# nicoloalbergoni/DeepLabV3Plus-Augmented-SuperResolution

Measured on AMD Instinct MI355X. Metric: augmented-copies/sec (fwd+realign+SR-iter) @512x512, higher is better.
Workload: dtype f32 (pointwise GEMMs: operands split into f16 hi+lo, hi*hi+hi*lo+lo*hi on f16 MFMA, f32 accumulate)

## Files before the change

### deeplabv3plus-augmented-superresolution_amd/csrc/sr.hip

```cpp
#include "asr_warp_device.h"

namespace {

constexpr int kTileX = 32, kTileY = 8;

struct SrDims {
    int batch, n, H, W, h, w, f;
};

__global__ __launch_bounds__(256) void sr_init_kernel(const float* __restrict__ y, float* __restrict__ x,
                                                      SrDims d, float scale_y, float scale_x) {
    const int X = blockIdx.x * kTileX + threadIdx.x;
    const int Y = blockIdx.y * kTileY + threadIdx.y;
    const int b = blockIdx.z;
    if (X >= d.W || Y >= d.H) return;
    const float* src = y + (int64_t)b * d.n * d.h * d.w;
    const AsrLerp ly = asr_half_pixel(Y, scale_y, d.h);
    const AsrLerp lx = asr_half_pixel(X, scale_x, d.w);
    const float tl = src[ly.lo * d.w + lx.lo], tr = src[ly.lo * d.w + lx.hi];
    const float bl = src[ly.hi * d.w + lx.lo], br = src[ly.hi * d.w + lx.hi];
    const float top = tl + (tr - tl) * lx.t;
    const float bot = bl + (br - bl) * lx.t;
    x[((int64_t)b * d.H + Y) * d.W + X] = top + (bot - top) * ly.t;
}

#if defined(ASR_DIAG_KFWD_CHECK) || defined(ASR_DIAG_KFWD_NOPK)
__device__ __forceinline__ float dg_mul(float x, float y) { float z; asm volatile("v_mul_f32 %0, %1, %2" : "=v"(z) : "v"(x), "v"(y)); return z; }
__device__ __forceinline__ float dg_add(float x, float y) { float z; asm volatile("v_add_f32 %0, %1, %2" : "=v"(z) : "v"(x), "v"(y)); return z; }
__device__ __forceinline__ float dg_sub(float x, float y) { float z; asm volatile("v_sub_f32 %0, %1, %2" : "=v"(z) : "v"(x), "v"(y)); return z; }
#endif
#ifndef ASR_DIAG_KFWD_NOPK
#define ASR_DIAG_KFWD_NOPK 0
#endif
constexpr int kGrPadX = 32, kGrPadY = 2;
__host__ __device__ inline size_t sr_gr_plane_elems(int H, int W) { return (size_t)(H + 2 * kGrPadY) * (size_t)(W + 2 * kGrPadX); }
typedef float asr_f2u __attribute__((ext_vector_type(2), aligned(4)));

__device__ __forceinline__ float sr_bilinear_bordered(const float* __restrict__ plane, int WP, int H, int W, float ix, float iy) {
    const float xf = floorf(ix), yf = floorf(iy);
    const int x0 = (int)__builtin_amdgcn_fmed3f(xf, -2.0f, (float)W), y0 = (int)__builtin_amdgcn_fmed3f(yf, -2.0f, (float)H);
    const unsigned off = (unsigned)(__mul24(y0, WP * 4) + (kGrPadY * WP * 4 + kGrPadX * 4) + x0 * 4);
    const char* const base = reinterpret_cast<const char*>(plane);
    const char* const base_next = base + WP * 4;
    const asr_f2u top = *reinterpret_cast<const asr_f2u*>(base + off);
    const asr_f2u bot = *reinterpret_cast<const asr_f2u*>(base_next + off);
#ifdef ASR_DIAG_KFWD_WAIT
    asm volatile("s_waitcnt vmcnt(0)" ::: "memory");
#endif
#if ASR_DIAG_KFWD_NOPK & 2
    const float wxl = dg_sub(dg_add(xf, 1.0f), ix), wxh = dg_sub(ix, xf);
    const float vyf = dg_add(dg_mul(wxl, top.x), dg_mul(wxh, top.y));
    const float vyc = dg_add(dg_mul(wxl, bot.x), dg_mul(wxh, bot.y));
    return dg_add(dg_mul(dg_sub(dg_add(yf, 1.0f), iy), vyf), dg_mul(dg_sub(iy, yf), vyc));
// ... 282 lines not shown
            const float acc = v[o] + g * g;
            v[o] = acc;
            xn = xc - (g * alpha) / (sqrtf(acc) + st.c2);
            break;
        }
        case ASR_OPT_ADADELTA: {
            const float acc = v[o] * st.c0 + (g * g) * st.c1;
            v[o] = acc;
            const float au = m[o];
            const float upd = sqrtf(au + st.c2) * (1.0f / sqrtf(acc + st.c2)) * g;
            xn = xc - upd * alpha;
            m[o] = au * st.c0 + (upd * upd) * st.c1;
            break;
        }
        case ASR_OPT_ADAMAX: {
            float mm = m[o];
            mm = mm + (g - mm) * st.c0;
            const float vv = fmaxf(st.c1 * v[o], fabsf(g));
            m[o] = mm;
            v[o] = vv;
            xn = xc - alpha * (mm / (vv + st.c2));
            break;
        }
        default: {
            float mm = m[o], vv = v[o];
            mm = mm + (g - mm) * st.c0;
            vv = vv + (g * g - vv) * st.c1;
            m[o] = mm;
            v[o] = vv;
            float denom;
            if (st.flag) {
                const float vh = fmaxf(vhat[o], vv);
                vhat[o] = vh;
                denom = sqrtf(vh) + st.c2;
            } else {
                denom = sqrtf(vv) + st.c2;
            }
            xn = xc - (mm * alpha) / denom;
        }
    }
    x_new[o] = xn;
    if (x_bordered_out)
        x_bordered_out[(size_t)b * sr_gr_plane_elems(H, W) + (size_t)(Y + kGrPadY) * (W + 2 * kGrPadX) + (X + kGrPadX)] = xn;
}

constexpr int kBwdSplit = 4, kBwdPixX = 32, kBwdPixY = 2, kBwdPix = kBwdPixX * kBwdPixY;

constexpr int kGrRows = 16;

template <int LOG2F>
__global__ __launch_bounds__(256) void sr_grad_translate_kernel(const float* __restrict__ resid,
                                                                const float* __restrict__ inv_trans_tf,
                                                                float* __restrict__ gr_out, SrDims d, float two_lambda_df,
                                                                int n0, int cn) {
    const int slot = blockIdx.z;
    const int bn = (slot / cn) * d.n + n0 + (slot % cn);
    const int lane = threadIdx.x;
    const int cx = blockIdx.x * 64 + lane;
    const int cy0 = (blockIdx.y * 4 + __builtin_amdgcn_readfirstlane(threadIdx.y)) * kGrRows;
    const int H = d.H, W = d.W, f = d.f, lw = d.w, lh = d.h;
    const int ph0 = f / 2 - 1, ph1 = f / 2;
    const int WP = W + 2 * kGrPadX;
    const float* r = resid + (int64_t)bn * lh * lw;
    const AsrTf8 it = asr_load_tf(inv_trans_tf + (int64_t)bn * 8);
    float* const out = gr_out + (size_t)slot * sr_gr_plane_elems(H, W) + (size_t)kGrPadY * WP + kGrPadX;
    const bool col_ok = cx < W;
    const bool pure_translation = (it.a0 == 1.0f && it.a1 == 0.0f && it.b0 == 0.0f && it.b1 == 1.0f &&
                                   it.c0 == 0.0f && it.c1 == 0.0f);
    if (pure_translation) {
        const SrAxisTap ax = sr_axis_tap<LOG2F>(col_ok ? cx : 0, it.a2, W, f, ph0, ph1);
        const int c0 = max(ax.l0, 0), c1 = max(ax.l1, 0);
        const bool ok0 = ax.l0 >= 0, ok1 = ax.l1 >= 0;
        const SrAxisTap ayv = sr_axis_tap<LOG2F>(min(cy0 + lane, H - 1), it.b2, H, f, ph0, ph1);
        auto xblend = [&](int L) -> float {
            const float* row = r + L * lw;
            const float a = (two_lambda_df * row[c0]) * 0.25f, b = (two_lambda_df * row[c1]) * 0.25f;
            return ax.wl * (ok0 ? a : 0.0f) + ax.wh * (ok1 ? b : 0.0f);
        };
        int la = -1, lb = -1;
        float va = 0.0f, vb = 0.0f;
        auto h_of = [&](int L) -> float {
            if (L < 0) return 0.0f;
            if (L == lb) return vb;
            if (L == la) return va;
            la = lb; va = vb;
            lb = L; vb = xblend(L);
            return vb;
        };
        const int rows = min(kGrRows, H - cy0);
        for (int j = 0; j < rows; ++j) {
            const float wl = __builtin_bit_cast(float, __builtin_amdgcn_readlane(__builtin_bit_cast(int, ayv.wl), j));
            const float wh = __builtin_bit_cast(float, __builtin_amdgcn_readlane(__builtin_bit_cast(int, ayv.wh), j));
            const int l0 = __builtin_amdgcn_readlane(ayv.l0, j), l1 = __builtin_amdgcn_readlane(ayv.l1, j);
            const float h0 = h_of(l0), h1 = h_of(l1);
            if (col_ok) out[(cy0 + j) * WP + cx] = wl * h0 + wh * h1;
        }
    } else {
        auto gt_at = [&](int ly, int lx) -> float {
            const bool ok = (ly >= 0) & (lx >= 0);
            const float v = (two_lambda_df * r[ok ? ly * lw + lx : 0]) * 0.25f;
            return ok ? v : 0.0f;
        };
        auto rd_gt = [&](int yt, int xt) -> float {
            return gt_at(sr_gt_index<LOG2F>(yt, H, f, ph0, ph1), sr_gt_index<LOG2F>(xt, W, f, ph0, ph1));
        };
        for (int j = 0; j < kGrRows; ++j) {
            const int cy = cy0 + j;
            if (cy < H && col_ok) out[cy * WP + cx] = asr_tf_sample(it, rd_gt, cx, cy);
        }
    }
}

template <int LOG2F, bool WTV>
__global__ __launch_bounds__(256) void sr_backward_adam_kernel(
    const float* __restrict__ x, float* __restrict__ x_new, const float* __restrict__ resid,
    const float* __restrict__ inv_rot_tf, const float* __restrict__ inv_trans_tf,
    float* __restrict__ m, float* __restrict__ v, float* __restrict__ vhat,
    const float* __restrict__ alphas , float* __restrict__ grad_out,
    SrDims d, float two_lambda_df, float lambda_tv, float two_lambda_l2, float lambda_l1, SrStep st, SrTvW tw) {
    extern __shared__ float contrib[];
    const int X = blockIdx.x * kBwdPixX + threadIdx.x;
    const int Y = blockIdx.y * kBwdPixY + threadIdx.y;
    const int b = blockIdx.z;
    const int grp = threadIdx.z;
    const int pix = threadIdx.y * kBwdPixX + threadIdx.x;
    const bool in_image = (X < d.W) & (Y < d.H);
    const int H = d.H, W = d.W, f = d.f, lw = d.w, lh = d.h;
    const int ph0 = f / 2 - 1, ph1 = f / 2;

    auto contribution = [&](int n) -> float {
        float g_df = 0.0f;
        const int bn = b * d.n + n;
        const AsrTf8 ir = asr_load_tf(inv_rot_tf + (int64_t)bn * 8);
        const float* r = resid + (int64_t)bn * lh * lw;
        const AsrTf8 it = asr_load_tf(inv_trans_tf + (int64_t)bn * 8);
        auto gt_at = [&](int ly, int lx) -> float {
            const bool ok = (ly >= 0) & (lx >= 0);
            const float v = (two_lambda_df * r[ok ? ly * lw + lx : 0]) * 0.25f;
            return ok ? v : 0.0f;
        };
        const bool pure_translation = (it.a0 == 1.0f && it.a1 == 0.0f && it.b0 == 0.0f && it.b1 == 1.0f &&
                                       it.c0 == 0.0f && it.c1 == 0.0f);
        if (pure_translation) {
// ... 109 lines not shown
    for (int i = threadIdx.x; i < n; i += 64) {
        const float* t = inv_rot_tf + ((int64_t)b * n + i) * 8;
        ok = ok && t[6] == 0.0f && t[7] == 0.0f;
    }
    const bool all = __builtin_amdgcn_ballot_w64(!ok) == 0;
    if (threadIdx.x == 0) flags[b] = all ? 1 : 0;
}

template <bool WTV>
__global__ __launch_bounds__(256) void sr_backward_gather_kernel(
    const float* __restrict__ x, float* __restrict__ x_new, const float* __restrict__ gr_planes,
    const float* __restrict__ inv_rot_tf, float* __restrict__ m, float* __restrict__ v, float* __restrict__ vhat,
    const float* __restrict__ alphas, float* __restrict__ grad_out, SrDims d, float lambda_tv, float two_lambda_l2,
    float lambda_l1, SrStep st, float* __restrict__ x_bordered_out, float* __restrict__ acc, int n0, int cn,
    const int* __restrict__ affine_flags, SrTvW tw) {
    const int X = blockIdx.x * 64 + threadIdx.x;
    const int Y = blockIdx.y * 4 + threadIdx.y;
    const int b = blockIdx.z;
    const int H = d.H, W = d.W, WP = W + 2 * kGrPadX;
    if (X >= W || Y >= H) return;
    const size_t plane = sr_gr_plane_elems(H, W);
    const float* const planes = gr_planes + (size_t)b * cn * plane;
    const float* const tfs = inv_rot_tf + ((int64_t)b * d.n + n0) * 8;
    const float fx = (float)X, fy = (float)Y;
    const int64_t o = ((int64_t)b * H + Y) * W + X;
    float g_df = (n0 == 0) ? 0.0f : acc[o];
    int n = 0;
    if (affine_flags[b]) {
        for (; n + 8 <= cn; n += 8) g_df = sr_gather_chunk<8, true>(g_df, tfs + n * 8, planes + n * plane, plane, WP, H, W, fx, fy);
        if (n + 4 <= cn) { g_df = sr_gather_chunk<4, true>(g_df, tfs + n * 8, planes + n * plane, plane, WP, H, W, fx, fy); n += 4; }
        for (; n < cn; ++n) g_df = sr_gather_chunk<1, true>(g_df, tfs + n * 8, planes + n * plane, plane, WP, H, W, fx, fy);
    } else {
        for (; n < cn; ++n) g_df = sr_gather_chunk<1, false>(g_df, tfs + n * 8, planes + n * plane, plane, WP, H, W, fx, fy);
    }
    if (n0 + cn < d.n) { acc[o] = g_df; return; }
    sr_prior_and_update<WTV>(x, x_new, m, v, vhat, alphas, grad_out, d, b, X, Y, g_df, lambda_tv, two_lambda_l2, lambda_l1, st,
                             tw, x_bordered_out);
}

typedef void (*SrBwdKernel)(const float*, float*, const float*, const float*, const float*, float*, float*, float*,
                            const float*, float*, SrDims, float, float, float, float, SrStep, SrTvW);

template <bool WTV>
SrBwdKernel sr_backward_kernel_of(int f) {
    switch (f) {
        case 2: return sr_backward_adam_kernel<1, WTV>;
        case 4: return sr_backward_adam_kernel<2, WTV>;
        case 8: return sr_backward_adam_kernel<3, WTV>;
        default: return sr_backward_adam_kernel<0, WTV>;
    }
}
SrBwdKernel sr_backward_kernel_for(int f, bool wtv) { return wtv ? sr_backward_kernel_of<true>(f) : sr_backward_kernel_of<false>(f); }

typedef void (*SrGradTranslateKernel)(const float*, const float*, float*, SrDims, float, int, int);
SrGradTranslateKernel sr_grad_translate_kernel_for(int f) {
    switch (f) {
        case 2: return sr_grad_translate_kernel<1>;
        case 4: return sr_grad_translate_kernel<2>;
        case 8: return sr_grad_translate_kernel<3>;
        default: return sr_grad_translate_kernel<0>;
    }
}

__global__ __launch_bounds__(256) void sr_loss_df_kernel(const float* __restrict__ resid, double* __restrict__ out,
                                                         int64_t per_image) {
    const int b = blockIdx.y;
    const float* r = resid + (int64_t)b * per_image;
    double acc = 0.0;
    for (int64_t p = (int64_t)blockIdx.x * 256 + threadIdx.x; p < per_image; p += (int64_t)gridDim.x * 256) {
        const float t = r[p];
        acc += (double)(t * t);
    }
    acc = asr_wave_sum(acc);
    if ((threadIdx.x & 63) == 0) atomicAdd(out + (int64_t)b * 4 + 0, acc);
}

template <bool WTV>
__global__ __launch_bounds__(256) void sr_loss_prior_kernel(const float* __restrict__ x, double* __restrict__ out,
                                                            int H, int W, SrStep st, SrTvW tw) {
    const int b = blockIdx.y;
    const float* img = x + (int64_t)b * H * W;
    double tv = 0.0, l2 = 0.0, l1 = 0.0;
    const int64_t total = (int64_t)H * W;
    for (int64_t p = (int64_t)blockIdx.x * 256 + threadIdx.x; p < total; p += (int64_t)gridDim.x * 256) {
        const int X = (int)(p % W), Y = (int)(p / W);
        const float xc = img[p];
        if (st.prior == ASR_PRIOR_BTV) {
            for (int hh = -st.btv_shift; hh <= st.btv_shift; ++hh)
                for (int vv = 0; vv <= st.btv_shift; ++vv) {
                    const int xs = X - hh, ys = Y - vv;
                    const float sv = (xs >= 0 && xs < W && ys >= 0 && ys < H) ? img[(int64_t)ys * W + xs] : 0.0f;
                    tv += (double)st.btv_w[abs(hh) + vv] * (double)fabsf(xc - sv);
                }
        } else if (WTV) {
            const float dy = (Y < H - 1) ? img[p + W] - xc : 0.0f;
            const float dx = (X < W - 1) ? img[p + 1] - xc : 0.0f;
            const int64_t q = (int64_t)b * tw.stride + p;
            tv += (double)(tw.wy[q] * fabsf(dy) + tw.wx[q] * fabsf(dx));
        } else {
            const float dy = (Y < H - 1) ? img[p + W] - xc : 0.0f;
            const float dx = (X < W - 1) ? img[p + 1] - xc : 0.0f;
            tv += (double)(fabsf(dy) + fabsf(dx));
        }
        l2 += (double)(xc * xc);
        l1 += (double)fabsf(xc);
    }
    tv = asr_wave_sum(tv);
// ... 67 lines not shown
    };
    V val;
    float ix, iy;
    const bool ok = asr_tf_map(tr, (float)X, (float)Y, ix, iy);
    const float xf = floorf(ix), yf = floorf(iy);
    const int x0 = asr_coord_to_int(xf), y0 = asr_coord_to_int(yf);
    const bool pure_translation = (tt.a0 == 1.0f) & (tt.a1 == 0.0f) & (tt.b0 == 0.0f) & (tt.b1 == 1.0f) &
                                  (tt.c0 == 0.0f) & (tt.c1 == 0.0f);
    const float jx0 = (float)x0 + tt.a2, jx1 = (float)(x0 + 1) + tt.a2;
    const float jy0 = (float)y0 + tt.b2, jy1 = (float)(y0 + 1) + tt.b2;
    const float fx0 = floorf(jx0), fx1 = floorf(jx1), fy0 = floorf(jy0), fy1 = floorf(jy1);
    const int cx0 = asr_coord_to_int(fx0), cx1 = asr_coord_to_int(fx1);
    const int cy0 = asr_coord_to_int(fy0), cy1 = asr_coord_to_int(fy1);
    if (ok && pure_translation && cx1 == cx0 + 1 && cy1 == cy0 + 1) {
        V uv[3][3];
#pragma unroll
        for (int a = 0; a < 3; ++a)
#pragma unroll
            for (int c = 0; c < 3; ++c) uv[a][c] = rd_up(cy0 + a, cx0 + c);
        const float wxl0 = (fx0 + 1.0f) - jx0, wxh0 = jx0 - fx0, wxl1 = (fx1 + 1.0f) - jx1, wxh1 = jx1 - fx1;
        const float wyl0 = (fy0 + 1.0f) - jy0, wyh0 = jy0 - fy0, wyl1 = (fy1 + 1.0f) - jy1, wyh1 = jy1 - fy1;
        auto Tq = [&](int a, int c, float wxl, float wxh, float wyl, float wyh) -> V {
            const V vyf = wxl * uv[a][c] + wxh * uv[a][c + 1];
            const V vyc = wxl * uv[a + 1][c] + wxh * uv[a + 1][c + 1];
            return wyl * vyf + wyh * vyc;
        };
        const bool vx0 = x0 >= 0 && x0 < W, vx1 = x0 + 1 >= 0 && x0 + 1 < W;
        const bool vy0 = y0 >= 0 && y0 < H, vy1 = y0 + 1 >= 0 && y0 + 1 < H;
        const V v00 = (vy0 && vx0) ? Tq(0, 0, wxl0, wxh0, wyl0, wyh0) : zero;
        const V v01 = (vy0 && vx1) ? Tq(0, 1, wxl1, wxh1, wyl0, wyh0) : zero;
        const V v10 = (vy1 && vx0) ? Tq(1, 0, wxl0, wxh0, wyl1, wyh1) : zero;
        const V v11 = (vy1 && vx1) ? Tq(1, 1, wxl1, wxh1, wyl1, wyh1) : zero;
        const float wxl = (xf + 1.0f) - ix, wxh = ix - xf;
        const V vyf = wxl * v00 + wxh * v01;
        const V vyc = wxl * v10 + wxh * v11;
        val = ((yf + 1.0f) - iy) * vyf + (iy - yf) * vyc;
    } else {
        val = asr_tf_sample(tr, rd_tr, X, Y);
    }
    return val;
}
__device__ __forceinline__ float sr_realign_copy_value(const float* __restrict__ y, const float* __restrict__ trans_tf,
                                                       const float* __restrict__ rot_tf, int bn, int X, int Y, int H, int W,
                                                       int lh, int lw, float scale_y, float scale_x) {
    const float* const src[1] = {y + (int64_t)bn * lh * lw};
    return sr_realign_copy_value<1>(src, trans_tf, rot_tf, bn, X, Y, H, W, lh, lw, scale_y, scale_x).v[0];
}

template <int MODE>
__global__ __launch_bounds__(256) void sr_realign_kernel(const float* __restrict__ y, float* __restrict__ out_a,
                                                         float* __restrict__ out_b,
                                                         const float* __restrict__ trans_tf ,
                                                         const float* __restrict__ rot_tf ,
                                                         SrDims d, float scale_y, float scale_x) {
    const int X = blockIdx.x * kTileX + threadIdx.x;
    const int Y = blockIdx.y * kTileY + threadIdx.y;
    const int b = blockIdx.z;
    if (X >= d.W || Y >= d.H) return;
    const int H = d.H, W = d.W, lh = d.h, lw = d.w;
    float acc_sum = 0.0f, acc_max = 0.0f;
    for (int n = 0; n < d.n; ++n) {
        const float val = sr_realign_copy_value(y, trans_tf, rot_tf, b * d.n + n, X, Y, H, W, lh, lw, scale_y, scale_x);
        if (MODE != 0) acc_max = (n == 0) ? val : fmaxf(acc_max, val);
        if (MODE != 1) acc_sum += val;
    }
    const int64_t o = ((int64_t)b * H + Y) * W + X;
    if (MODE == 0) out_a[o] = acc_sum / (float)d.n;
    if (MODE == 1) out_a[o] = acc_max;
    if (MODE == 2) { out_a[o] = acc_max; out_b[o] = acc_sum / (float)d.n; }
}

constexpr int kSelX = 32, kSelY = 2, kSelPix = kSelX * kSelY;
constexpr int kSelMaxQ = 8;
constexpr int kSelLdsMax = 160 * 1024;
constexpr int kSelMaxCopies = kSelLdsMax / (kSelPix * (int)sizeof(unsigned));

struct SrSelect {
    int num_q, trim_k;
    int lo[kSelMaxQ], hi[kSelMaxQ];
    float t[kSelMaxQ];
};

__device__ __forceinline__ unsigned sr_sel_key(float v) {
    const unsigned u = __float_as_uint(v == 0.0f ? 0.0f : v);
    return u ^ ((u >> 31) ? 0xffffffffu : 0x80000000u);
}
__device__ __forceinline__ float sr_sel_value(unsigned k) {
    return __uint_as_float(k ^ ((k >> 31) ? 0x80000000u : 0xffffffffu));
}
__device__ __forceinline__ unsigned sr_sel_rank(const unsigned* col, int n, int rank) {
    unsigned prefix = 0u;
    for (int bit = 31; bit >= 0; --bit) {
        const unsigned cand = prefix | (1u << bit);
        int below = 0;
#pragma unroll 8
        for (int i = 0; i < n; ++i) below += (col[i * kSelPix] < cand) ? 1 : 0;
        prefix = (below <= rank) ? cand : prefix;
    }
    return prefix;
}

__global__ __launch_bounds__(kSelPix) void sr_realign_select_kernel(const float* __restrict__ y, float* __restrict__ out_q,
                                                                    float* __restrict__ out_trim,
                                                                    const float* __restrict__ trans_tf,
                                                                    const float* __restrict__ rot_tf, SrDims d, SrSelect sel,
                                                                    int tiles_x, float scale_y, float scale_x) {
    extern __shared__ unsigned sel_keys[];
    const int tile_y = blockIdx.x / tiles_x, tile_x = blockIdx.x - tile_y * tiles_x;
    const int X = tile_x * kSelX + threadIdx.x;
    const int Y = tile_y * kSelY + threadIdx.y;
    const int b = blockIdx.z;
    if (X >= d.W || Y >= d.H) return;
    const int H = d.H, W = d.W, lh = d.h, lw = d.w, n = d.n;
    unsigned* col = sel_keys + threadIdx.y * kSelX + threadIdx.x;
    for (int i = 0; i < n; ++i) {
        const float val = sr_realign_copy_value(y, trans_tf, rot_tf, b * n + i, X, Y, H, W, lh, lw, scale_y, scale_x);
        col[i * kSelPix] = sr_sel_key(val);
    }
    const int64_t plane = (int64_t)d.batch * H * W;
    const int64_t o = ((int64_t)b * H + Y) * W + X;
    for (int j = 0; j < sel.num_q; ++j) {
        const int lo = sel.lo[j], hi = sel.hi[j];
// ... 155 lines not shown
        if (walk == 0) {
            fnv = (float)cnt;
            m = (cnt > 0) ? acc / fnv : 0.0f;
            if (out_nv) out_nv[o] = fnv;
            if (out_mean) out_mean[o] = m;
        } else {
            out_var[o] = (fnv > 0.0f) ? acc / fnv : 0.0f;
        }
    }
}

int check_dims(const char* fn, int batch, int n, int H, int W, int h, int w, SrDims* d) {
    ASR_REQUIRE(batch > 0 && n > 0 && H > 0 && W > 0 && h > 0 && w > 0, "%s: bad shape batch=%d n=%d %dx%d <- %dx%d",
                fn, batch, n, H, W, h, w);
    ASR_REQUIRE((int64_t)batch * n <= 65535, "%s: batch*n=%lld exceeds 65535 (grid.z)", fn, (long long)batch * n);
    const int f = H / h;
    ASR_UNSUPPORTED(f * h != H || f * w != W || f < 2 || (f & 1),
                    "%s: output %dx%d must be an even integer multiple of the feature size %dx%d", fn, H, W, h, w);
    d->batch = batch; d->n = n; d->H = H; d->W = W; d->h = h; d->w = w; d->f = f;
    return ASR_OK;
}

int prepare_backward(const SrDims& d, bool wtv) {
    const size_t lds = sizeof(float) * (size_t)d.n * 64;
    ASR_UNSUPPORTED(lds > 160 * 1024, "asr_sr: num_aug=%d needs %zu bytes of LDS in the backward kernel (max 640 copies)", d.n, lds);
    static AsrDeviceOnce once[8];
    const int idx = (d.f == 2 ? 1 : (d.f == 4 ? 2 : (d.f == 8 ? 3 : 0))) + (wtv ? 4 : 0);
    if (lds > 64 * 1024)
        ASR_HIP_CHECK(asr_allow_dynamic_lds(once[idx], reinterpret_cast<const void*>(sr_backward_kernel_for(d.f, wtv)), 160 * 1024));
    return ASR_OK;
}
dim3 gr_grid(const SrDims& d, int cn) {
    return dim3((unsigned)asr_cdiv(d.W, 64), (unsigned)asr_cdiv(d.H, 4 * kGrRows), (unsigned)(d.batch * cn));
}
constexpr size_t kPlaneBytesMax = (size_t)1 << 30;
int sr_plane_chunk(int batch, int n, int H, int W, int requested) {
    if (requested > 0) return requested < n ? requested : n;
    const size_t per_copy = sizeof(float) * (size_t)batch * sr_gr_plane_elems(H, W);
    const size_t fit = kPlaneBytesMax / per_copy > 0 ? kPlaneBytesMax / per_copy : 1;
    if ((size_t)n <= fit) return n;
    const int chunks = (int)(((size_t)n + fit - 1) / fit);
    return (n + chunks - 1) / chunks;
}
size_t sr_workspace_bytes(int batch, int n, int H, int W, int h, int w, int chunk) {
    return sizeof(float) * ((size_t)batch * n * h * w + 2 * (size_t)batch * H * W +
                            ((size_t)batch * chunk + batch) * sr_gr_plane_elems(H, W)) + sizeof(int) * (size_t)batch;
}
dim3 gather_grid(const SrDims& d) {
    return dim3((unsigned)asr_cdiv(d.W, 64), (unsigned)asr_cdiv(d.H, 4), (unsigned)d.batch);
}
dim3 bwd_grid(const SrDims& d) { return dim3((unsigned)asr_cdiv(d.W, kBwdPixX), (unsigned)asr_cdiv(d.H, kBwdPixY), (unsigned)d.batch); }
const dim3 kBwdBlock(kBwdPixX, kBwdPixY, kBwdSplit);
size_t bwd_lds(const SrDims& d) { return sizeof(float) * (size_t)d.n * kBwdPix; }
dim3 hr_grid(const SrDims& d) { return dim3((unsigned)asr_cdiv(d.W, kTileX), (unsigned)asr_cdiv(d.H, kTileY), (unsigned)d.batch); }
dim3 lr_grid(const SrDims& d) { return dim3((unsigned)asr_cdiv(d.w, kTileX), (unsigned)asr_cdiv(d.h, kTileY), (unsigned)(d.batch * d.n)); }
const dim3 kBlock(kTileX, kTileY);

}

extern "C" int asr_sr_init_target_f32(const float* y, float* x, int batch, int n, int H, int W, int h, int w,
                                      asr_stream_t stream) {
    ASR_REQUIRE(y && x, "asr_sr_init_target_f32: null pointer");
    SrDims d;
    ASR_REQUIRE(batch > 0 && n > 0 && H > 0 && W > 0 && h > 0 && w > 0, "asr_sr_init_target_f32: bad shape");
    d.batch = batch; d.n = n; d.H = H; d.W = W; d.h = h; d.w = w; d.f = 0;
    const float sy = (float)h / (float)H, sx = (float)w / (float)W;
    hipLaunchKernelGGL(sr_init_kernel, hr_grid(d), kBlock, 0, asr_stream(stream), y, x, d, sy, sx);
    ASR_LAUNCH_CHECK();
    return ASR_OK;
}

extern "C" int asr_sr_forward_residual_f32(const float* x, const float* y, const float* rot_tf, const float* trans_tf,
                                           float* resid, int batch, int n, int H, int W, int h, int w,
                                           asr_stream_t stream) {
    ASR_REQUIRE(x && y && rot_tf && trans_tf && resid, "asr_sr_forward_residual_f32: null pointer");
    SrDims d;
    int rc = check_dims("asr_sr_forward_residual_f32", batch, n, H, W, h, w, &d);
    if (rc != ASR_OK) return rc;
    hipLaunchKernelGGL(sr_forward_residual_kernel<false>, lr_grid(d), kBlock, 0, asr_stream(stream), x, y, rot_tf, trans_tf,
                       resid, d);
    ASR_LAUNCH_CHECK();
    return ASR_OK;
}

namespace {

int make_step(const char* fn, const asr_sr_config* cfg, bool need_update, const float* m, const float* v, const float* vhat,
              SrStep* st) {
    ASR_REQUIRE(cfg, "%s: null config", fn);
    ASR_REQUIRE(cfg->optimizer >= ASR_OPT_ADAM && cfg->optimizer <= ASR_OPT_ADAMAX, "%s: unknown optimizer %d", fn, cfg->optimizer);
    ASR_REQUIRE(cfg->prior == ASR_PRIOR_TV || cfg->prior == ASR_PRIOR_BTV, "%s: unknown prior %d", fn, cfg->prior);
    st->optimizer = cfg->optimizer; st->flag = cfg->flag; st->c0 = cfg->c0; st->c1 = cfg->c1; st->c2 = cfg->c2;
    st->prior = cfg->prior; st->btv_shift = 0;
    for (int k = 0; k < 9; ++k) st->btv_w[k] = 0.0f;
    if (cfg->prior == ASR_PRIOR_BTV) {
        ASR_REQUIRE(cfg->btv_shift >= 1 && cfg->btv_shift <= 4, "%s: btv_shift %d outside [1, 4]", fn, cfg->btv_shift);
        st->btv_shift = cfg->btv_shift;
        for (int k = 0; k <= 2 * cfg->btv_shift; ++k) st->btv_w[k] = powf(cfg->btv_alpha, (float)k);
    }
    if (need_update) {
        bool ok = true;
        switch (cfg->optimizer) {
            case ASR_OPT_ADAM: ok = m && v && (vhat || !cfg->flag); break;
            case ASR_OPT_SGD: ok = m || cfg->c0 == 0.0f; break;
            case ASR_OPT_ADAGRAD: ok = v != nullptr; break;
            default: ok = m && v; break;
// ... 122 lines not shown
extern "C" int asr_sr_loss_terms_f64(const float* x, const float* resid, double* terms, int batch, int n, int H, int W,
                                     int h, int w, asr_stream_t stream) {
    const asr_sr_config c = adam_tv_config(0.f, 0.f, 0.f, 0);
    return asr_sr_loss_terms_cfg_f64(x, resid, terms, batch, n, H, W, h, w, &c, stream);
}

extern "C" size_t asr_sr_solve_workspace_bytes(int batch, int n, int H, int W, int h, int w) {
    return sr_workspace_bytes(batch, n, H, W, h, w, sr_plane_chunk(batch, n, H, W, 0));
}

extern "C" size_t asr_sr_solve_workspace_bytes_cfg(int batch, int n, int H, int W, int h, int w, const asr_sr_config* cfg) {
    return sr_workspace_bytes(batch, n, H, W, h, w, sr_plane_chunk(batch, n, H, W, cfg ? cfg->plane_chunk : 0));
}

namespace {
int sr_solve_impl(const char* fn, float* x, const float* y, const float* rot_tf, const float* trans_tf, const float* inv_rot_tf,
                  const float* inv_trans_tf, float* m, float* v, float* vhat, const float* alphas, int num_iter,
                  double* last_loss_terms, void* workspace, size_t workspace_bytes, int batch, int n, int H, int W, int h, int w,
                  float lambda_df, float lambda_tv, float lambda_l2, float lambda_l1, const asr_sr_config* cfg,
                  const SrTvWArg& wa, asr_stream_t stream) {
    ASR_REQUIRE(x && y && rot_tf && trans_tf && inv_rot_tf && inv_trans_tf && alphas && workspace, "%s: null pointer", fn);
    ASR_REQUIRE(num_iter >= 0, "%s: num_iter < 0", fn);
    SrDims d;
    int rc = check_dims(fn, batch, n, H, W, h, w, &d);
    if (rc != ASR_OK) return rc;
    SrStep st;
    rc = make_step(fn, cfg, true, m, v, vhat, &st);
    if (rc != ASR_OK) return rc;
    SrTvW tw;
    rc = make_tv_weights(fn, cfg, wa, H, W, &tw);
    if (rc != ASR_OK) return rc;
    ASR_REQUIRE(cfg->plane_chunk >= 0, "%s: plane_chunk %d < 0", fn, cfg->plane_chunk);
    const int chunk = sr_plane_chunk(batch, n, H, W, cfg->plane_chunk);
    ASR_REQUIRE((int64_t)batch * chunk <= 65535, "%s: batch*chunk=%lld exceeds 65535 (grid.z)", fn, (long long)batch * chunk);
    const size_t need = sr_workspace_bytes(batch, n, H, W, h, w, chunk);
    if (workspace_bytes < need) {
        asr_set_error("%s: workspace %zu < required %zu bytes", fn, workspace_bytes, need);
        return ASR_ERR_WORKSPACE;
    }
    hipStream_t s = asr_stream(stream);
    float* resid = static_cast<float*>(workspace);
    float* x_alt = resid + (size_t)batch * n * h * w;
    float* cur = x;
    float* nxt = x_alt;
    float* const acc = x_alt + (size_t)batch * H * W;
    float* const gr = acc + (size_t)batch * H * W;
    const SrGradTranslateKernel gr_kernel = sr_grad_translate_kernel_for(d.f);
    float* const xb = gr + (size_t)batch * chunk * sr_gr_plane_elems(H, W);
    int* const affine_flags = reinterpret_cast<int*>(xb + (size_t)batch * sr_gr_plane_elems(H, W));
    if (num_iter > 0) {
        hipLaunchKernelGGL(sr_affine_flags_kernel, dim3((unsigned)batch), dim3(64), 0, s, inv_rot_tf, affine_flags, n);
        ASR_LAUNCH_CHECK();
    }
    if (num_iter > 0) {
        const size_t pe = sr_gr_plane_elems(H, W);
        ASR_HIP_CHECK(hipMemsetAsync(gr, 0, sizeof(float) * ((size_t)batch * chunk + batch) * pe, s));
        const size_t wp = (size_t)W + 2 * kGrPadX;
        for (int b = 0; b < batch; ++b)
            ASR_HIP_CHECK(hipMemcpy2DAsync(xb + b * pe + kGrPadY * wp + kGrPadX, wp * sizeof(float), x + (size_t)b * H * W,
                                           (size_t)W * sizeof(float), (size_t)W * sizeof(float), (size_t)H,
                                           hipMemcpyDeviceToDevice, s));
    }
    for (int it = 0; it < num_iter; ++it) {
        hipLaunchKernelGGL(sr_forward_residual_kernel<true>, lr_grid(d), kBlock, 0, s, xb, y, rot_tf, trans_tf, resid, d);
        ASR_LAUNCH_CHECK();
        if (last_loss_terms && it == num_iter - 1) {
            rc = sr_loss_terms_impl(fn, cur, resid, last_loss_terms, batch, n, H, W, h, w, cfg, wa, stream);
            if (rc != ASR_OK) return rc;
        }
        for (int n0 = 0; n0 < n; n0 += chunk) {
            const int cn = n - n0 < chunk ? n - n0 : chunk;
            hipLaunchKernelGGL(gr_kernel, gr_grid(d, cn), dim3(64, 4), 0, s, resid, inv_trans_tf, gr, d, 2.0f * lambda_df, n0, cn);
            ASR_LAUNCH_CHECK();
            const auto bwd_kernel = wa.weighted ? sr_backward_gather_kernel<true> : sr_backward_gather_kernel<false>;
            hipLaunchKernelGGL(bwd_kernel, gather_grid(d), dim3(64, 4), 0, s, cur, nxt, gr, inv_rot_tf, m, v, vhat,
                               alphas + (size_t)it * batch, (float*)nullptr, d, lambda_tv, 2.0f * lambda_l2, lambda_l1, st, xb,
                               acc, n0, cn, affine_flags, tw);
            ASR_LAUNCH_CHECK();
        }
        float* t = cur; cur = nxt; nxt = t;
    }
    if (cur != x) ASR_HIP_CHECK(hipMemcpyAsync(x, cur, sizeof(float) * (size_t)batch * H * W, hipMemcpyDeviceToDevice, s));
    return ASR_OK;
}

__global__ __launch_bounds__(256) SR_NO_PK_F32 void sr_tv_edge_weights_kernel(const float* __restrict__ guide, float* __restrict__ wy,
                                                                              float* __restrict__ wx, int H, int W, float beta) {
    const int X = blockIdx.x * kTileX + threadIdx.x;
    const int Y = blockIdx.y * kTileY + threadIdx.y;
    if (X >= W || Y >= H) return;
    const int64_t o = ((int64_t)blockIdx.z * H + Y) * W + X;
    const float* c = guide + o * 3;
    const float c0 = c[0], c1 = c[1], c2 = c[2];
    float vy = 1.0f, vx = 1.0f;
    if (Y < H - 1) {
        const float* q = c + (int64_t)W * 3;
        const float a0 = q[0] - c0, a1 = q[1] - c1, a2 = q[2] - c2;
        const float dd = (a0 * a0 + a1 * a1) + a2 * a2;
        vy = 1.0f / (1.0f + beta * dd);
    }
    if (X < W - 1) {
        const float a0 = c[3] - c0, a1 = c[4] - c1, a2 = c[5] - c2;
        const float dd = (a0 * a0 + a1 * a1) + a2 * a2;
        vx = 1.0f / (1.0f + beta * dd);
    }
    wy[o] = vy;
    wx[o] = vx;
}
}

extern "C" int asr_tv_edge_weights_f32(const float* guide, float* wy, float* wx, int batch, int H, int W, float beta,
                                       asr_stream_t stream) {
    ASR_REQUIRE(guide && wy && wx, "asr_tv_edge_weights_f32: null pointer");
    ASR_REQUIRE(batch > 0 && batch <= 65535 && H > 0 && W > 0, "asr_tv_edge_weights_f32: bad shape batch=%d %dx%d", batch, H, W);
    ASR_REQUIRE(beta >= 0.0f && beta < __builtin_inff(), "asr_tv_edge_weights_f32: beta=%g must be finite and >= 0", (double)beta);
    SrDims d;
    d.batch = batch; d.n = 1; d.H = H; d.W = W; d.h = H; d.w = W; d.f = 0;
    hipLaunchKernelGGL(sr_tv_edge_weights_kernel, hr_grid(d), kBlock, 0, asr_stream(stream), guide, wy, wx, H, W, beta);
    ASR_LAUNCH_CHECK();
    return ASR_OK;
}

extern "C" int asr_sr_solve_cfg_f32(float* x, const float* y, const float* rot_tf, const float* trans_tf,
                                    const float* inv_rot_tf, const float* inv_trans_tf, float* m, float* v, float* vhat,
                                    const float* alphas, int num_iter, double* last_loss_terms, void* workspace,
                                    size_t workspace_bytes, int batch, int n, int H, int W, int h, int w,
                                    float lambda_df, float lambda_tv, float lambda_l2, float lambda_l1,
                                    const asr_sr_config* cfg, asr_stream_t stream) {
    return sr_solve_impl("asr_sr_solve_cfg_f32", x, y, rot_tf, trans_tf, inv_rot_tf, inv_trans_tf, m, v, vhat, alphas, num_iter,
                         last_loss_terms, workspace, workspace_bytes, batch, n, H, W, h, w, lambda_df, lambda_tv, lambda_l2,
                         lambda_l1, cfg, kNoTvW, stream);
}

extern "C" int asr_sr_solve_wtv_f32(float* x, const float* y, const float* rot_tf, const float* trans_tf,
                                    const float* inv_rot_tf, const float* inv_trans_tf, float* m, float* v, float* vhat,
                                    const float* alphas, int num_iter, double* last_loss_terms, void* workspace,
                                    size_t workspace_bytes, int batch, int n, int H, int W, int h, int w,
                                    float lambda_df, float lambda_tv, float lambda_l2, float lambda_l1,
                                    const asr_sr_config* cfg, const float* wy, const float* wx, int w_shared,
                                    asr_stream_t stream) {
    const SrTvWArg wa = {wy, wx, w_shared, true};
    return sr_solve_impl("asr_sr_solve_wtv_f32", x, y, rot_tf, trans_tf, inv_rot_tf, inv_trans_tf, m, v, vhat, alphas, num_iter,
                         last_loss_terms, workspace, workspace_bytes, batch, n, H, W, h, w, lambda_df, lambda_tv, lambda_l2,
                         lambda_l1, cfg, wa, stream);
}

extern "C" int asr_sr_solve_f32(float* x, const float* y, const float* rot_tf, const float* trans_tf,
                                const float* inv_rot_tf, const float* inv_trans_tf, float* m, float* v, float* vhat,
                                const float* alphas, int num_iter, double* last_loss_terms, void* workspace,
                                size_t workspace_bytes, int batch, int n, int H, int W, int h, int w,
                                float lambda_df, float lambda_tv, float lambda_l2, float lambda_l1,
                                float one_minus_beta1, float one_minus_beta2, float epsilon, int amsgrad,
                                asr_stream_t stream) {
    const asr_sr_config c = adam_tv_config(one_minus_beta1, one_minus_beta2, epsilon, amsgrad);
    return asr_sr_solve_cfg_f32(x, y, rot_tf, trans_tf, inv_rot_tf, inv_trans_tf, m, v, vhat, alphas, num_iter,
                                last_loss_terms, workspace, workspace_bytes, batch, n, H, W, h, w, lambda_df, lambda_tv,
                                lambda_l2, lambda_l1, &c, stream);
}

static int realign_common(int mode, const float* y, float* out_a, float* out_b, const float* trans_tf, const float* rot_tf,
                          int batch, int n, int H, int W, int h, int w, asr_stream_t stream) {
    ASR_REQUIRE(y && out_a && trans_tf && rot_tf && (mode != 2 || out_b), "asr_realign: null pointer");
    ASR_REQUIRE(batch > 0 && batch <= 65535 && n > 0 && H > 0 && W > 0 && h > 0 && w > 0, "asr_realign: bad shape");
    SrDims d;
    d.batch = batch; d.n = n; d.H = H; d.W = W; d.h = h; d.w = w; d.f = 0;
    const float sy = (float)h / (float)H, sx = (float)w / (float)W;
    hipStream_t s = asr_stream(stream);
    if (mode == 1) hipLaunchKernelGGL(sr_realign_kernel<1>, hr_grid(d), kBlock, 0, s, y, out_a, out_b, trans_tf, rot_tf, d, sy, sx);
    else if (mode == 0) hipLaunchKernelGGL(sr_realign_kernel<0>, hr_grid(d), kBlock, 0, s, y, out_a, out_b, trans_tf, rot_tf, d, sy, sx);
    else hipLaunchKernelGGL(sr_realign_kernel<2>, hr_grid(d), kBlock, 0, s, y, out_a, out_b, trans_tf, rot_tf, d, sy, sx);
    ASR_LAUNCH_CHECK();
    return ASR_OK;
}

extern "C" int asr_realign_max_f32(const float* y, float* out, const float* trans_tf, const float* rot_tf, int batch,
                                   int n, int H, int W, int h, int w, asr_stream_t stream) {
    return realign_common(1, y, out, nullptr, trans_tf, rot_tf, batch, n, H, W, h, w, stream);
}

extern "C" int asr_realign_mean_f32(const float* y, float* out, const float* trans_tf, const float* rot_tf, int batch,
                                    int n, int H, int W, int h, int w, asr_stream_t stream) {
    return realign_common(0, y, out, nullptr, trans_tf, rot_tf, batch, n, H, W, h, w, stream);
}

extern "C" int asr_realign_max_mean_f32(const float* y, float* out_max, float* out_mean, const float* trans_tf,
                                        const float* rot_tf, int batch, int n, int H, int W, int h, int w,
                                        asr_stream_t stream) {
    return realign_common(2, y, out_max, out_mean, trans_tf, rot_tf, batch, n, H, W, h, w, stream);
}

extern "C" int asr_realign_select_max_copies(void) { return kSelMaxCopies; }

extern "C" int asr_realign_select_f32(const float* y, float* out_q, float* out_trim, const int* lo_rank, const int* hi_rank,
                                      const float* t, int num_q, int trim_k, const float* trans_tf, const float* rot_tf,
                                      int batch, int n, int H, int W, int h, int w, asr_stream_t stream) {
    ASR_REQUIRE(y && trans_tf && rot_tf, "asr_realign_select_f32: null pointer");
    ASR_REQUIRE(num_q >= 0 && num_q <= kSelMaxQ, "asr_realign_select_f32: num_q=%d (0..%d)", num_q, kSelMaxQ);
    ASR_REQUIRE(num_q > 0 || out_trim, "asr_realign_select_f32: nothing to compute (num_q = 0 and no out_trim)");
    ASR_REQUIRE(num_q == 0 || (out_q && lo_rank && hi_rank && t), "asr_realign_select_f32: null pointer");
    ASR_REQUIRE(batch > 0 && batch <= 65535 && n > 0 && H > 0 && W > 0 && h > 0 && w > 0, "asr_realign_select_f32: bad shape");
    ASR_UNSUPPORTED(n > kSelMaxCopies, "asr_realign_select_f32: n=%d copies, at most %d (256 bytes of LDS per copy, 160 KiB per workgroup)",
                    n, kSelMaxCopies);
    SrSelect sel = {};
    sel.num_q = num_q;
    for (int j = 0; j < num_q; ++j) {
        ASR_REQUIRE(lo_rank[j] >= 0 && lo_rank[j] <= hi_rank[j] && hi_rank[j] <= n - 1,
                    "asr_realign_select_f32: ranks[%d] = (%d, %d) need 0 <= lo <= hi <= n - 1 = %d", j, lo_rank[j], hi_rank[j], n - 1);
        sel.lo[j] = lo_rank[j]; sel.hi[j] = hi_rank[j]; sel.t[j] = t[j];
    }
    ASR_REQUIRE(trim_k >= 0 && 2 * (int64_t)trim_k < n, "asr_realign_select_f32: trim_k=%d needs 0 <= 2k < n = %d", trim_k, n);
    ASR_REQUIRE(out_trim || trim_k == 0, "asr_realign_select_f32: trim_k=%d without out_trim", trim_k);
    sel.trim_k = trim_k;
    const int64_t tiles_x = asr_cdiv(W, kSelX), tiles = tiles_x * asr_cdiv(H, kSelY);
    ASR_REQUIRE(tiles <= 0x7fffffff, "asr_realign_select_f32: %dx%d output exceeds the grid", H, W);
    SrDims d;
    d.batch = batch; d.n = n; d.H = H; d.W = W; d.h = h; d.w = w; d.f = 0;
    const float sy = (float)h / (float)H, sx = (float)w / (float)W;
    const size_t lds = sizeof(unsigned) * (size_t)n * kSelPix;
    static AsrDeviceOnce once;
    if (lds > 64 * 1024)
        ASR_HIP_CHECK(asr_allow_dynamic_lds(once, reinterpret_cast<const void*>(sr_realign_select_kernel), kSelLdsMax));
    hipLaunchKernelGGL(sr_realign_select_kernel, dim3((unsigned)tiles, 1, (unsigned)batch), dim3(kSelX, kSelY), lds,
                       asr_stream(stream), y, out_q, out_trim, trans_tf, rot_tf, d, sel, (int)tiles_x, sy, sx);
    ASR_LAUNCH_CHECK();
// ... 73 lines not shown
```

Before: 2158.

## Split realign into translate-plane pass and rotation gather for translation-only batches

For batches whose transforms decompose into a pure translation followed by a rotation, realign now runs in two stages. First it materialises per-copy translated, upsampled planes with row caching into pooled scratch memory, in chunks. A gather kernel then applies the rotation with a bilinear lookup and reduces max and mean, and the original per-pixel kernel skips those batches through a flags array. The SR gradient kernel also skips output rows whose taps are all out of range when only one chunk is used. This trades redundant per-pixel composite sampling for extra scratch traffic, added launches and a stream-ordered memory pool.

```diff
diff --git a/deeplabv3plus-augmented-superresolution_amd/csrc/sr.hip b/deeplabv3plus-augmented-superresolution_amd/csrc/sr.hip
--- a/deeplabv3plus-augmented-superresolution_amd/csrc/sr.hip
+++ b/deeplabv3plus-augmented-superresolution_amd/csrc/sr.hip
@@ -1,4 +1,5 @@
 #include "asr_warp_device.h"
+#include <mutex>
 
 namespace {
 
@@ -387,7 +388,7 @@
 __global__ __launch_bounds__(256) void sr_grad_translate_kernel(const float* __restrict__ resid,
                                                                 const float* __restrict__ inv_trans_tf,
                                                                 float* __restrict__ gr_out, SrDims d, float two_lambda_df,
-                                                                int n0, int cn) {
+                                                                int n0, int cn, int skip_zero_rows) {
     const int slot = blockIdx.z;
     const int bn = (slot / cn) * d.n + n0 + (slot % cn);
     const int lane = threadIdx.x;
@@ -423,7 +424,10 @@
             return vb;
         };
         const int rows = min(kGrRows, H - cy0);
+        const unsigned long long zero_rows =
+            skip_zero_rows ? __builtin_amdgcn_ballot_w64(ayv.l0 < 0 && ayv.l1 < 0 && ayv.wl == ayv.wl && ayv.wh == ayv.wh) : 0ull;
         for (int j = 0; j < rows; ++j) {
+            if ((zero_rows >> j) & 1ull) continue;
             const float wl = __builtin_bit_cast(float, __builtin_amdgcn_readlane(__builtin_bit_cast(int, ayv.wl), j));
             const float wh = __builtin_bit_cast(float, __builtin_amdgcn_readlane(__builtin_bit_cast(int, ayv.wh), j));
             const int l0 = __builtin_amdgcn_readlane(ayv.l0, j), l1 = __builtin_amdgcn_readlane(ayv.l1, j);
@@ -639,7 +643,7 @@
 }
 SrBwdKernel sr_backward_kernel_for(int f, bool wtv) { return wtv ? sr_backward_kernel_of<true>(f) : sr_backward_kernel_of<false>(f); }
 
-typedef void (*SrGradTranslateKernel)(const float*, const float*, float*, SrDims, float, int, int);
+typedef void (*SrGradTranslateKernel)(const float*, const float*, float*, SrDims, float, int, int, int);
 SrGradTranslateKernel sr_grad_translate_kernel_for(int f) {
     switch (f) {
         case 2: return sr_grad_translate_kernel<1>;
@@ -813,11 +817,13 @@
                                                          float* __restrict__ out_b,
                                                          const float* __restrict__ trans_tf ,
                                                          const float* __restrict__ rot_tf ,
-                                                         SrDims d, float scale_y, float scale_x) {
+                                                         SrDims d, float scale_y, float scale_x,
+                                                         const int* __restrict__ plane_flags) {
     const int X = blockIdx.x * kTileX + threadIdx.x;
     const int Y = blockIdx.y * kTileY + threadIdx.y;
     const int b = blockIdx.z;
     if (X >= d.W || Y >= d.H) return;
+    if (plane_flags && plane_flags[b]) return;
     const int H = d.H, W = d.W, lh = d.h, lw = d.w;
     float acc_sum = 0.0f, acc_max = 0.0f;
     for (int n = 0; n < d.n; ++n) {
@@ -829,6 +835,179 @@
     if (MODE == 0) out_a[o] = acc_sum / (float)d.n;
     if (MODE == 1) out_a[o] = acc_max;
     if (MODE == 2) { out_a[o] = acc_max; out_b[o] = acc_sum / (float)d.n; }
+}
+
+__global__ __launch_bounds__(64) void sr_realign_flags_kernel(const float* __restrict__ trans_tf, const float* __restrict__ rot_tf,
+                                                              int* __restrict__ flags, int n) {
+    const int b = blockIdx.x;
+    bool ok = true;
+    for (int i = threadIdx.x; i < n; i += 64) {
+        const float* r = rot_tf + ((int64_t)b * n + i) * 8;
+        const float* t = trans_tf + ((int64_t)b * n + i) * 8;
+        ok = ok && r[6] == 0.0f && r[7] == 0.0f && t[0] == 1.0f && t[1] == 0.0f && t[3] == 0.0f && t[4] == 1.0f &&
+             t[6] == 0.0f && t[7] == 0.0f;
+    }
+    const bool all = __builtin_amdgcn_ballot_w64(!ok) == 0;
+    if (threadIdx.x == 0) flags[b] = all ? 1 : 0;
+}
+
+struct SrUpTap {
+    int lo, hi;
+    float t;
+    bool ok;
+};
+__device__ __forceinline__ SrUpTap sr_up_tap(int u, int size, float scale, int in_size) {
+    SrUpTap r;
+    r.ok = (u >= 0 && u < size);
+    const AsrLerp l = asr_half_pixel(r.ok ? u : 0, scale, in_size);
+    r.lo = l.lo; r.hi = l.hi; r.t = l.t;
+    return r;
+}
+
+__global__ __launch_bounds__(256) void sr_realign_planes_kernel(const float* __restrict__ y, const float* __restrict__ trans_tf,
+                                                                float* __restrict__ planes, const int* __restrict__ flags,
+                                                                SrDims d, float scale_y, float scale_x, int n0, int cn) {
+    const int slot = blockIdx.z;
+    const int b = slot / cn;
+    if (!flags[b]) return;
+    const int bn = b * d.n + n0 + (slot % cn);
+    const int lane = threadIdx.x;
+    const int cx = blockIdx.x * 64 + lane;
+    const int cy0 = (blockIdx.y * 4 + __builtin_amdgcn_readfirstlane(threadIdx.y)) * kGrRows;
+    const int H = d.H, W = d.W, lh = d.h, lw = d.w;
+    if (cy0 >= H) return;
+    const int WP = W + 2 * kGrPadX;
+    const float* const src = y + (int64_t)bn * lh * lw;
+    float* const out = planes + (size_t)slot * sr_gr_plane_elems(H, W) + (size_t)kGrPadY * WP + kGrPadX;
+    const bool col_ok = cx < W;
+    const bool col_st = cx < W + 2;
+    const int rows = min(kGrRows, H - cy0);
+    if ((int)blockIdx.x * 64 < W) {
+        const AsrTf8 tt = asr_load_tf(trans_tf + (int64_t)bn * 8);
+        const float jx = (float)(col_ok ? cx : 0) + tt.a2;
+        const float fx = floorf(jx);
+        const float wxl = (fx + 1.0f) - jx, wxh = jx - fx;
+        const int ux = asr_coord_to_int(fx);
+        const SrUpTap x0 = sr_up_tap(ux, W, scale_x, lw), x1 = sr_up_tap(ux + 1, W, scale_x, lw);
+        const float jy = (float)min(cy0 + lane, H - 1) + tt.b2;
+        const float fy = floorf(jy);
+        const float wylv = (fy + 1.0f) - jy, wyhv = jy - fy;
+        const int uyv = asr_coord_to_int(fy);
+        const SrUpTap y0v = sr_up_tap(uyv, H, scale_y, lh), y1v = sr_up_tap(uyv + 1, H, scale_y, lh);
+        int la = -1, lb = -1;
+        float va0 = 0.0f, va1 = 0.0f, vb0 = 0.0f, vb1 = 0.0f;
+        auto lr_row = [&](int L, float& o0, float& o1) {
+            if (L == lb) { o0 = vb0; o1 = vb1; return; }
+            if (L == la) { o0 = va0; o1 = va1; return; }
+            la = lb; va0 = vb0; va1 = vb1;
+            const float* row = src + L * lw;
+            const float l0 = row[x0.lo], r0 = row[x0.hi], l1 = row[x1.lo], r1 = row[x1.hi];
+            lb = L; vb0 = l0 + (r0 - l0) * x0.t; vb1 = l1 + (r1 - l1) * x1.t;
+            o0 = vb0; o1 = vb1;
+        };
+        int ua = -1, ub = -1;
+        float wa0 = 0.0f, wa1 = 0.0f, wb0 = 0.0f, wb1 = 0.0f;
+        auto up_row = [&](int u, int lo, int hi, float t, float& o0, float& o1) {
+            if (u < 0 || u >= H) { o0 = 0.0f; o1 = 0.0f; return; }
+            if (u == ub) { o0 = wb0; o1 = wb1; return; }
+            if (u == ua) { o0 = wa0; o1 = wa1; return; }
+            ua = ub; wa0 = wb0; wa1 = wb1;
+            float top0, top1, bot0, bot1;
+            lr_row(lo, top0, top1);
+            lr_row(hi, bot0, bot1);
+            const float u0 = top0 + (bot0 - top0) * t, u1 = top1 + (bot1 - top1) * t;
+            ub = u; wb0 = x0.ok ? u0 : 0.0f; wb1 = x1.ok ? u1 : 0.0f;
+            o0 = wb0; o1 = wb1;
+        };
+        auto rl_i = [](int v, int j) -> int { return __builtin_amdgcn_readlane(v, j); };
+        auto rl_f = [](float v, int j) -> float {
+            return __builtin_bit_cast(float, __builtin_amdgcn_readlane(__builtin_bit_cast(int, v), j));
+        };
+        for (int j = 0; j < rows; ++j) {
+            const float wyl = rl_f(wylv, j), wyh = rl_f(wyhv, j);
+            const int uy = rl_i(uyv, j);
+            float a0, a1, b0, b1;
+            up_row(uy, rl_i(y0v.lo, j), rl_i(y0v.hi, j), rl_f(y0v.t, j), a0, a1);
+            up_row(uy + 1, rl_i(y1v.lo, j), rl_i(y1v.hi, j), rl_f(y1v.t, j), b0, b1);
+            const float vyf = wxl * a0 + wxh * a1;
+            const float vyc = wxl * b0 + wxh * b1;
+            const float val = wyl * vyf + wyh * vyc;
+            if (col_st) out[(cy0 + j) * WP + cx] = col_ok ? val : 0.0f;
+        }
+    } else {
+        for (int j = 0; j < rows; ++j)
+            if (col_st) out[(cy0 + j) * WP + cx] = 0.0f;
+    }
+    const bool left = blockIdx.x == 0 && lane < 2;
+    for (int j = 0; j < rows; ++j)
+        if (left) out[(cy0 + j) * WP + lane - 2] = 0.0f;
+    if (cy0 == 0)
+        for (int r = -2; r < 0; ++r) {
+            if (col_st) out[r * WP + cx] = 0.0f;
+            if (left) out[r * WP + lane - 2] = 0.0f;
+        }
+    if (cy0 + kGrRows >= H)
+        for (int r = H; r < H + 2; ++r) {
+            if (col_st) out[r * WP + cx] = 0.0f;
+            if (left) out[r * WP + lane - 2] = 0.0f;
+        }
+}
+
+template <int K, int MODE>
+__device__ __forceinline__ void sr_realign_gather_chunk(float& acc_sum, float& acc_max, bool first, const float* __restrict__ rot_tf,
+                                                        const float* __restrict__ planes, size_t plane, int WP, int H, int W,
+                                                        float fx, float fy) {
+    AsrTf8 t[K];
+#pragma unroll
+    for (int u = 0; u < K; ++u) t[u] = asr_load_tf(rot_tf + u * 8);
+    float c[K];
+#pragma unroll
+    for (int u = 0; u < K; ++u) {
+        float ix, iy;
+        sr_map_affine(t[u], fx, fy, ix, iy);
+        c[u] = sr_bilinear_bordered(planes + u * plane, WP, H, W, ix, iy);
+    }
+#pragma unroll
+    for (int u = 0; u < K; ++u) {
+        if (MODE != 0) acc_max = (first && u == 0) ? c[u] : fmaxf(acc_max, c[u]);
+        if (MODE != 1) acc_sum += c[u];
+    }
+}
+
+template <int MODE>
+__global__ __launch_bounds__(256) void sr_realign_gather_kernel(const float* __restrict__ all_planes, float* out_a, float* out_b,
+                                                                const float* __restrict__ rot_tf, const int* __restrict__ flags,
+                                                                SrDims d, int n0, int cn) {
+    const int X = blockIdx.x * 64 + threadIdx.x;
+    const int Y = blockIdx.y * 4 + threadIdx.y;
+    const int b = blockIdx.z;
+    const int H = d.H, W = d.W, WP = W + 2 * kGrPadX;
+    if (X >= W || Y >= H) return;
+    if (!flags[b]) return;
+    const size_t plane = sr_gr_plane_elems(H, W);
+    const float* const planes = all_planes + (size_t)b * cn * plane;
+    const float* const tfs = rot_tf + ((int64_t)b * d.n + n0) * 8;
+    const float fx = (float)X, fy = (float)Y;
+    const int64_t o = ((int64_t)b * H + Y) * W + X;
+    float* const out_max = out_a;
+    float* const out_sum = (MODE == 2) ? out_b : out_a;
+    float acc_sum = 0.0f, acc_max = 0.0f;
+    if (n0 > 0) {
+        if (MODE != 0) acc_max = out_max[o];
+        if (MODE != 1) acc_sum = out_sum[o];
+    }
+    int n = 0;
+    for (; n + 8 <= cn; n += 8)
+        sr_realign_gather_chunk<8, MODE>(acc_sum, acc_max, n0 == 0 && n == 0, tfs + n * 8, planes + n * plane, plane, WP, H, W, fx, fy);
+    if (n + 4 <= cn) {
+        sr_realign_gather_chunk<4, MODE>(acc_sum, acc_max, n0 == 0 && n == 0, tfs + n * 8, planes + n * plane, plane, WP, H, W, fx, fy);
+        n += 4;
+    }
+    for (; n < cn; ++n)
+        sr_realign_gather_chunk<1, MODE>(acc_sum, acc_max, n0 == 0 && n == 0, tfs + n * 8, planes + n * plane, plane, WP, H, W, fx, fy);
+    const bool last = n0 + cn >= d.n;
+    if (MODE != 0) out_max[o] = acc_max;
+    if (MODE != 1) out_sum[o] = last ? acc_sum / (float)d.n : acc_sum;
 }
 
 constexpr int kSelX = 32, kSelY = 2, kSelPix = kSelX * kSelY;
@@ -1090,6 +1269,43 @@
 dim3 bwd_grid(const SrDims& d) { return dim3((unsigned)asr_cdiv(d.W, kBwdPixX), (unsigned)asr_cdiv(d.H, kBwdPixY), (unsigned)d.batch); }
 const dim3 kBwdBlock(kBwdPixX, kBwdPixY, kBwdSplit);
 size_t bwd_lds(const SrDims& d) { return sizeof(float) * (size_t)d.n * kBwdPix; }
+#ifndef ASR_REALIGN_CHUNK_COPIES
+#define ASR_REALIGN_CHUNK_COPIES 128
+#endif
+constexpr int kRealignChunkCopies = ASR_REALIGN_CHUNK_COPIES;
+int sr_realign_chunk(int batch, int n, int H, int W) {
+    const size_t per_copy = sizeof(float) * (size_t)batch * sr_gr_plane_elems(H, W);
+    size_t fit = kPlaneBytesMax / per_copy;
+    if (fit > (size_t)kRealignChunkCopies) fit = (size_t)kRealignChunkCopies;
+    if (fit > (size_t)(65535 / batch)) fit = (size_t)(65535 / batch);
+    if (fit == 0) return 0;
+    if ((size_t)n <= fit) return n;
+    const int chunks = (int)(((size_t)n + fit - 1) / fit);
+    return (n + chunks - 1) / chunks;
+}
+hipMemPool_t sr_scratch_pool() {
+    static std::mutex mu;
+    static hipMemPool_t pools[64] = {};
+    int dev = -1;
+    if (hipGetDevice(&dev) != hipSuccess || dev < 0 || dev >= 64) return nullptr;
+    std::lock_guard<std::mutex> guard(mu);
+    if (!pools[dev]) {
+        hipMemPoolProps props = {};
+        props.allocType = hipMemAllocationTypePinned;
+        props.handleTypes = hipMemHandleTypeNone;
+        props.location.type = hipMemLocationTypeDevice;
+        props.location.id = dev;
+        hipMemPool_t p = nullptr;
+        if (hipMemPoolCreate(&p, &props) != hipSuccess) {
+            (void)hipGetLastError();
+            return nullptr;
+        }
+        uint64_t keep = UINT64_MAX;
+        if (hipMemPoolSetAttribute(p, hipMemPoolAttrReleaseThreshold, &keep) != hipSuccess) (void)hipGetLastError();
+        pools[dev] = p;
+    }
+    return pools[dev];
+}
 dim3 hr_grid(const SrDims& d) { return dim3((unsigned)asr_cdiv(d.W, kTileX), (unsigned)asr_cdiv(d.H, kTileY), (unsigned)d.batch); }
 dim3 lr_grid(const SrDims& d) { return dim3((unsigned)asr_cdiv(d.w, kTileX), (unsigned)asr_cdiv(d.h, kTileY), (unsigned)(d.batch * d.n)); }
 const dim3 kBlock(kTileX, kTileY);
@@ -1318,6 +1534,7 @@
         hipLaunchKernelGGL(sr_affine_flags_kernel, dim3((unsigned)batch), dim3(64), 0, s, inv_rot_tf, affine_flags, n);
         ASR_LAUNCH_CHECK();
     }
+    const int one_chunk = chunk >= n ? 1 : 0;
     if (num_iter > 0) {
         const size_t pe = sr_gr_plane_elems(H, W);
         ASR_HIP_CHECK(hipMemsetAsync(gr, 0, sizeof(float) * ((size_t)batch * chunk + batch) * pe, s));
@@ -1336,7 +1553,8 @@
         }
         for (int n0 = 0; n0 < n; n0 += chunk) {
             const int cn = n - n0 < chunk ? n - n0 : chunk;
-            hipLaunchKernelGGL(gr_kernel, gr_grid(d, cn), dim3(64, 4), 0, s, resid, inv_trans_tf, gr, d, 2.0f * lambda_df, n0, cn);
+            hipLaunchKernelGGL(gr_kernel, gr_grid(d, cn), dim3(64, 4), 0, s, resid, inv_trans_tf, gr, d, 2.0f * lambda_df, n0, cn,
+                               one_chunk);
             ASR_LAUNCH_CHECK();
             const auto bwd_kernel = wa.weighted ? sr_backward_gather_kernel<true> : sr_backward_gather_kernel<false>;
             hipLaunchKernelGGL(bwd_kernel, gather_grid(d), dim3(64, 4), 0, s, cur, nxt, gr, inv_rot_tf, m, v, vhat,
@@ -1432,10 +1650,40 @@
     d.batch = batch; d.n = n; d.H = H; d.W = W; d.h = h; d.w = w; d.f = 0;
     const float sy = (float)h / (float)H, sx = (float)w / (float)W;
     hipStream_t s = asr_stream(stream);
-    if (mode == 1) hipLaunchKernelGGL(sr_realign_kernel<1>, hr_grid(d), kBlock, 0, s, y, out_a, out_b, trans_tf, rot_tf, d, sy, sx);
-    else if (mode == 0) hipLaunchKernelGGL(sr_realign_kernel<0>, hr_grid(d), kBlock, 0, s, y, out_a, out_b, trans_tf, rot_tf, d, sy, sx);
-    else hipLaunchKernelGGL(sr_realign_kernel<2>, hr_grid(d), kBlock, 0, s, y, out_a, out_b, trans_tf, rot_tf, d, sy, sx);
+    const size_t pe = sr_gr_plane_elems(H, W);
+    const int chunk = sr_realign_chunk(batch, n, H, W);
+    void* scratch = nullptr;
+    hipMemPool_t pool = nullptr;
+    if (pe * sizeof(float) < ((size_t)1 << 31) && H <= 4 * 65535 && W < (1 << 20) && chunk > 0) pool = sr_scratch_pool();
+    if (pool) {
+        const size_t bytes = sizeof(float) * (size_t)batch * chunk * pe + sizeof(int) * (size_t)batch;
+        if (hipMallocFromPoolAsync(&scratch, bytes, pool, s) != hipSuccess) {
+            (void)hipGetLastError();
+            scratch = nullptr;
+        }
+    }
+    int* flags = nullptr;
+    if (scratch) {
+        float* const planes = static_cast<float*>(scratch);
+        flags = reinterpret_cast<int*>(planes + (size_t)batch * chunk * pe);
+        hipLaunchKernelGGL(sr_realign_flags_kernel, dim3((unsigned)batch), dim3(64), 0, s, trans_tf, rot_tf, flags, n);
+        ASR_LAUNCH_CHECK();
+        for (int n0 = 0; n0 < n; n0 += chunk) {
+            const int cn = n - n0 < chunk ? n - n0 : chunk;
+            const dim3 pgrid((unsigned)asr_cdiv(W + 2, 64), (unsigned)asr_cdiv(H, 4 * kGrRows), (unsigned)(batch * cn));
+            hipLaunchKernelGGL(sr_realign_planes_kernel, pgrid, dim3(64, 4), 0, s, y, trans_tf, planes, flags, d, sy, sx, n0, cn);
+            ASR_LAUNCH_CHECK();
+            if (mode == 1) hipLaunchKernelGGL(sr_realign_gather_kernel<1>, gather_grid(d), dim3(64, 4), 0, s, planes, out_a, out_b, rot_tf, flags, d, n0, cn);
+            else if (mode == 0) hipLaunchKernelGGL(sr_realign_gather_kernel<0>, gather_grid(d), dim3(64, 4), 0, s, planes, out_a, out_b, rot_tf, flags, d, n0, cn);
+            else hipLaunchKernelGGL(sr_realign_gather_kernel<2>, gather_grid(d), dim3(64, 4), 0, s, planes, out_a, out_b, rot_tf, flags, d, n0, cn);
+            ASR_LAUNCH_CHECK();
+        }
+    }
+    if (mode == 1) hipLaunchKernelGGL(sr_realign_kernel<1>, hr_grid(d), kBlock, 0, s, y, out_a, out_b, trans_tf, rot_tf, d, sy, sx, flags);
+    else if (mode == 0) hipLaunchKernelGGL(sr_realign_kernel<0>, hr_grid(d), kBlock, 0, s, y, out_a, out_b, trans_tf, rot_tf, d, sy, sx, flags);
+    else hipLaunchKernelGGL(sr_realign_kernel<2>, hr_grid(d), kBlock, 0, s, y, out_a, out_b, trans_tf, rot_tf, d, sy, sx, flags);
     ASR_LAUNCH_CHECK();
+    if (scratch) ASR_HIP_CHECK(hipFreeAsync(scratch, s));
     return ASR_OK;
 }
 
```

Result: no change. 2166, median of 6 (+0.4%).
